# Fantom-foundation/go-txflow

Measured on AMD Instinct MI355X. Metric: verified+tallied TxVotes/sec, higher is better.
Workload: dtype u32

## Files before the change

go-txflow_amd/csrc/kernels_flow.hip:

```cpp
#include <algorithm>

#include "sha2.h"
#include "txv_device.h"
#include "txv_flow.h"
#include "lookback.h"

namespace {

constexpr int64_t kAminoMinSec = -62135596800LL;
constexpr int64_t kAminoMaxSec = 253402300800LL;
constexpr uint64_t kAddrSeed = 0x61646472ULL;
constexpr uint32_t kScanItems = 1024;

__device__ __forceinline__ uint64_t ld64u(const uint8_t* p) {
  const uintptr_t a = (uintptr_t)p;
  const uint32_t* q = reinterpret_cast<const uint32_t*>(a & ~(uintptr_t)3);
  const uint32_t s = (uint32_t)(a & 3u);
  const uint32_t w0 = q[0], w1 = q[1], w2 = q[2];
  return ((uint64_t)__builtin_amdgcn_alignbyte(w2, w1, s) << 32) | __builtin_amdgcn_alignbyte(w1, w0, s);
}

__device__ __forceinline__ bool key_eq(const uint8_t* a, const uint8_t* b, uint32_t n) {
  uint32_t i = 0;
  for (; i + 8 <= n; i += 8)
    if (ld64u(a + i) != ld64u(b + i)) return false;
  if (i < n) {
    const uint64_t m = (1ull << (8 * (n - i))) - 1ull;
    if ((ld64u(a + i) ^ ld64u(b + i)) & m) return false;
  }
  return true;
}

constexpr uint32_t kKeyRegBytes = 64;
struct KeyRegs {
  uint32_t w[16];
};
__device__ __forceinline__ void load_key(const uint8_t* p, uint32_t n, KeyRegs& k) {
  const uintptr_t a = (uintptr_t)p;
  const uint4* q = reinterpret_cast<const uint4*>(a & ~(uintptr_t)15);
  const uint32_t s = (uint32_t)(a & 15u);
  uint32_t raw[20];
#pragma unroll
  for (int c = 0; c < 5; ++c) {
    const uint4 v = (16u * c < s + n) ? q[c] : make_uint4(0, 0, 0, 0);
    raw[4 * c] = v.x; raw[4 * c + 1] = v.y; raw[4 * c + 2] = v.z; raw[4 * c + 3] = v.w;
// ... 271 lines not shown
  }
  if (t == 0) blk[nb] = total;
}

template <class Pred, class Act>
__global__ void __launch_bounds__(256) txv_k_scan_apply(Pred p, Act act, uint32_t n, const uint32_t* blk) {
  __shared__ uint32_t cnt[4][4];
  const uint32_t base = blockIdx.x * kScanItems + threadIdx.x;
  const int lane = threadIdx.x & 63, w = threadIdx.x >> 6;
  bool f[4];
  uint64_t m[4];
#pragma unroll
  for (int k = 0; k < 4; ++k) {
    f[k] = base + 256u * k < n && p(base + 256u * k);
    m[k] = __ballot(f[k]);
    if (lane == 0) cnt[k][w] = (uint32_t)__popcll(m[k]);
  }
  __syncthreads();
  uint32_t rank = blk[blockIdx.x];
  const uint64_t below = (1ull << lane) - 1ull;
#pragma unroll
  for (int k = 0; k < 4; ++k) {
    uint32_t before = 0, round = 0;
#pragma unroll
    for (int q = 0; q < 4; ++q) {
      before += q < w ? cnt[k][q] : 0u;
      round += cnt[k][q];
    }
    if (f[k]) act(base + 256u * k, rank + before + (uint32_t)__popcll(m[k] & below));
    rank += round;
  }
}

struct NewSetPred {
  FlowState fs;
  FlowBatch b;
  __device__ bool operator()(uint32_t i) const {
    const uint32_t e = b.entry[i];
    if (e == TXV_NONE) return false;
    const SetEntry& s = fs.tab[e];
    return s.state == TXV_SE_BATCH && s.first == i;
  }
};

struct NewSetAct {
  FlowState fs;
  FlowBatch b;
  __device__ void operator()(uint32_t i, uint32_t rank) const {
    const uint32_t slot = b.entry[i];
    SetEntry& e = fs.tab[slot];
    const uint32_t id = fs.ctr->n_sets + rank;
    e.state = TXV_SE_KEPT;
    if (id >= fs.max_txs) {
      atomicOr(&fs.ctr->err, TXV_FERR_SETS);
      e.id = TXV_NONE;
      return;
    }
    const uint32_t len = e.len, span = (len + 7u) & ~7u;
    uint64_t ko = (uint64_t)id * TXV_KEY_SLOT;
    if (len > TXV_KEY_SLOT) {
      const unsigned long long o = atomicAdd((unsigned long long*)&fs.ctr->key_used, (unsigned long long)span);
      if (o + span + 16 > fs.keys_cap) {
        atomicOr(&fs.ctr->err, TXV_FERR_KEYS);
        e.id = TXV_NONE;
        return;
      }
      ko = (uint64_t)fs.max_txs * TXV_KEY_SLOT + o;
    }
    const uint8_t* src = b.th + (e.key_off - 1);
    uint64_t* dst = reinterpret_cast<uint64_t*>(fs.keys + ko);
    for (uint32_t k = 0; k < span; k += 8)
      dst[k / 8] = ld64u(src + k) & (k + 8 <= len ? ~0ull : ((1ull << (8 * (len - k))) - 1ull));
    e.key_off = ko + 1;
    e.id = id;
    fs.set_entry[id] = slot;
    uint32_t* tk = fs.set_txkey + (size_t)id * 8;
    if (b.txkey) {
      const uint4* s4 = reinterpret_cast<const uint4*>(b.txkey + (size_t)i * 32);
      const uint4 a = s4[0], c = s4[1];
      tk[0] = a.x; tk[1] = a.y; tk[2] = a.z; tk[3] = a.w; tk[4] = c.x; tk[5] = c.y; tk[6] = c.z; tk[7] = c.w;
    } else {
#pragma unroll
      for (int j = 0; j < 8; ++j) tk[j] = 0;
    }
  }
};

__device__ __forceinline__ uint64_t cand_key(uint32_t stamp, uint32_t i) {
  return ((uint64_t)(0xFFFFFFFFu - stamp) << 32) | i;
}
__device__ __forceinline__ uint32_t cand_of(uint64_t c, uint32_t stamp) {
  return (uint32_t)(c >> 32) == 0xFFFFFFFFu - stamp ? (uint32_t)c : TXV_NONE;
}

constexpr uint8_t kReadCell = 1;
__global__ void __launch_bounds__(256) txv_k_tally_min(FlowState fs, FlowBatch b, uint32_t nb) {
  const uint32_t i = blockIdx.x * 256 + threadIdx.x;
  if (i == 0) {
    const uint32_t created = b.blk[nb];
    const uint32_t ns = fs.ctr->n_sets + created;
    fs.ctr->n_sets = ns > fs.max_txs ? fs.max_txs : ns;
    fs.ctr->n_stamped = 0;
    fs.ctr->ev_ticket = 0;
  }
  if (i >= b.n) return;
  const uint32_t e = b.entry[i];
  const uint32_t s = e == TXV_NONE ? TXV_NONE : fs.tab[e].id;
  b.set[i] = s;
  if (s == TXV_NONE || b.pre[i] != TXV_S_PENDING) return;
  if (b.ok[i] != 1) { b.status[i] = kReadCell; return; }
  TallyCell& c = fs.cell[(size_t)s * fs.n_vals + b.val[i]];
  if (c.acc != 0) { b.status[i] = kReadCell; return; }
  const uint64_t key = cand_key(b.stamp, i);
  const uint64_t old = atomicMin((unsigned long long*)&c.cand, (unsigned long long)key);
  uint8_t tf = 0;
  if (old < key) tf = kReadCell;
  else if (cand_of(old, b.stamp) != TXV_NONE) b.mark[(uint32_t)old] = 1;
  b.status[i] = tf;
}

__device__ __forceinline__ bool pending_in_set(const FlowBatch& b, uint32_t i) {
  return b.pre[i] == TXV_S_PENDING && b.set[i] != TXV_NONE;
}

__device__ __forceinline__ bool sig_eq_arena(const FlowState& fs, const FlowBatch& b, uint32_t i, uint32_t r) {
  uint32_t d = 0;
#pragma unroll
  for (int j = 0; j < 16; ++j) d |= b.sig[(size_t)j * b.n_pad + i] ^ fs.arena_sig[(size_t)j * fs.max_accepted + r];
  return d == 0;
}
__device__ __forceinline__ bool sig_eq_votes(const FlowBatch& b, uint32_t i, uint32_t f) {
  uint32_t d = 0;
// ... 208 lines not shown
    b.ev_host[rank] = e;
  }
};

__global__ void __launch_bounds__(256) txv_k_status_out(FlowState fs, FlowBatch b) {
  const uint32_t base = blockIdx.x * kScanItems + threadIdx.x;
  uint32_t c = 0;
#pragma unroll
  for (int k = 0; k < 4; ++k) {
    const uint32_t i = base + 256u * k;
    if (i >= b.n) continue;
    const uint8_t p = b.pre[i];
    uint8_t st = p;
    if (p == TXV_S_PENDING) {
      const uint32_t s = b.set[i];
      if (s == TXV_NONE) {
        st = TXV_S_INVALID_SIGNATURE;
      } else {
        st = b.status[i];
        if (st == TXV_S_ADDED) {
          const uint32_t x = fs.set_cross[s];
          if (x != TXV_NO_CROSS && i >= x) st |= TXV_S_FIRED;
        }
      }
    }
    b.status_host[i] = st;
    c += b.ev_flag[i] != 0;
  }
  uint32_t total;
  (void)block_excl_scan(c, &total);
  if (threadIdx.x == 0) b.blk[blockIdx.x] = total;
}

__global__ void __launch_bounds__(256) txv_k_event_top(FlowState fs, FlowBatch b, uint32_t nb) {
  const uint32_t t = threadIdx.x;
  const uint32_t per = (nb + 255) / 256;
  const uint32_t lo = min(t * per, nb), hi = min(lo + per, nb);
  uint32_t s = 0;
  for (uint32_t j = lo; j < hi; ++j) s += b.blk[j];
  uint32_t total;
  uint32_t run = block_excl_scan(s, &total);
  for (uint32_t j = lo; j < hi; ++j) {
    const uint32_t v = b.blk[j];
    b.blk[j] = run;
    run += v;
  }
  if (t == 0) {
    b.blk[nb] = total;
    FlowSummary sm;
    sm.n_sets = fs.ctr->n_sets;
    sm.n_events = total;
    sm.arena_used = min(fs.ctr->arena_used, fs.max_accepted);
    sm.err = fs.ctr->err;
    sm.key_used = fs.ctr->key_used;
    *b.summary_host = sm;
  }
}

constexpr uint32_t kFusedEventTiles = 128;
__global__ void __launch_bounds__(256) txv_k_status_events(FlowState fs, FlowBatch b, uint32_t n_tiles) {
  const uint32_t tile = take_tile(&fs.ctr->ev_ticket);
  const uint32_t base = tile * kScanItems + threadIdx.x;
  bool f[4];
#pragma unroll
  for (int k = 0; k < 4; ++k) {
    const uint32_t i = base + 256u * k;
    f[k] = false;
    if (i >= b.n) continue;
    const uint8_t p = b.pre[i];
    uint8_t st = p;
    if (p == TXV_S_PENDING) {
      const uint32_t s = b.set[i];
      if (s == TXV_NONE) {
        st = TXV_S_INVALID_SIGNATURE;
      } else {
        st = b.status[i];
        if (st == TXV_S_ADDED) {
          const uint32_t x = fs.set_cross[s];
          if (x != TXV_NO_CROSS && i >= x) st |= TXV_S_FIRED;
        }
      }
    }
    b.status_host[i] = st;
    f[k] = b.ev_flag[i] != 0;
  }
  uint32_t rank[4], total;
  tile_scan(f, rank, b.ev_tiles, tile, b.stamp, &fs.ctr->err, TXV_FERR_LOOKBACK, &total);
#pragma unroll
  for (int k = 0; k < 4; ++k) {
    if (!f[k]) continue;
    const uint32_t i = base + 256u * k, s = b.set[i];
    FlowEvent e;
    e.vote_index = i;
    e.tx_index = s;
    e.sum = fs.set_sum[s];
    b.ev_host[rank[k]] = e;
  }
  if (tile + 1 == n_tiles && threadIdx.x == 0) {
    FlowSummary sm;
    sm.n_sets = fs.ctr->n_sets;
    sm.n_events = total;
    sm.arena_used = min(fs.ctr->arena_used, fs.max_accepted);
    sm.err = __hip_atomic_load(&fs.ctr->err, __ATOMIC_RELAXED, __HIP_MEMORY_SCOPE_AGENT);
    sm.key_used = fs.ctr->key_used;
    *b.summary_host = sm;
  }
}

__global__ void __launch_bounds__(256) txv_k_reset_sets(FlowState fs, int keep_ids) {
  const uint32_t ns = fs.ctr->n_sets;
  const uint64_t cells = (uint64_t)ns * fs.n_vals;
  const uint64_t stride = (uint64_t)gridDim.x * 256;
  for (uint64_t c = (uint64_t)blockIdx.x * 256 + threadIdx.x; c < cells; c += stride)
    *reinterpret_cast<uint64_t*>(&fs.cell[c].acc) = 0;
  for (uint64_t s = (uint64_t)blockIdx.x * 256 + threadIdx.x; s < ns; s += stride) {
    fs.set_sum[s] = 0;
    if (!keep_ids) {
      SetEntry& e = fs.tab[fs.set_entry[s]];
      e.h = 0; e.len = 0; e.key_off = 0; e.first = 0; e.id = 0; e.state = TXV_SE_EMPTY;
    }
  }
}

__global__ void __launch_bounds__(256) txv_k_init_cells(FlowState fs, uint64_t cells, int clear_acc) {
  const uint64_t stride = (uint64_t)gridDim.x * 256;
  for (uint64_t c = (uint64_t)blockIdx.x * 256 + threadIdx.x; c < cells; c += stride) {
    fs.cell[c].cand = ~0ull;
    if (clear_acc) *reinterpret_cast<uint64_t*>(&fs.cell[c].acc) = 0;
  }
}

__global__ void txv_k_reset_counters(FlowState fs, int keep_ids) {
  if (!keep_ids) {
    fs.ctr->n_sets = 0;
    fs.ctr->n_digested = 0;
    fs.ctr->key_used = 0;
    fs.ctr->err = 0;
  } else {
    fs.ctr->err &= ~TXV_FERR_ARENA;
  }
  fs.ctr->arena_used = 0;
}

__global__ void __launch_bounds__(256) txv_k_lookup(FlowState fs, const uint8_t* keys, const uint32_t* off,
                                                    const uint32_t* len, uint32_t n, uint32_t* out_id) {
  const uint32_t q = blockIdx.x * 256 + threadIdx.x;
  if (q >= n) return;
  const uint8_t* kp = keys + off[q];
  const uint32_t l = len[q];
  const uint64_t h = txv_hash::hash_chunks(l, fs.hash_seed, [&](uint32_t k) { return ld64u(kp + k); });
  uint32_t id = TXV_NONE;
  for (uint32_t slot = (uint32_t)h & fs.tab_mask, probes = 0; probes <= fs.tab_mask; slot = (slot + 1) & fs.tab_mask, ++probes) {
    const SetEntry& e = fs.tab[slot];
    if (e.state == TXV_SE_EMPTY) break;
    if (e.state == TXV_SE_KEPT && e.h == h && e.len == l && key_eq(fs.keys + (e.key_off - 1), kp, l)) {
      id = e.id;
      break;
    }
  }
  out_id[q] = id;
}

__global__ void __launch_bounds__(256) txv_k_gather(FlowState fs, const uint32_t* ids, uint32_t n, int64_t* out_sum,
                                                    uint32_t* out_txkey, AccRow* out_rows) {
  const uint64_t t = (uint64_t)blockIdx.x * 256 + threadIdx.x;
  const uint32_t q = (uint32_t)(t / fs.n_vals), v = (uint32_t)(t % fs.n_vals);
  if (q >= n) return;
  const uint32_t id = ids[q];
  const bool ok = id != TXV_NONE && id < fs.max_txs;
  if (v == 0) {
    if (out_sum) out_sum[q] = ok ? fs.set_sum[id] : 0;
    if (out_txkey)
      for (int j = 0; j < 8; ++j) out_txkey[(size_t)q * 8 + j] = ok ? fs.set_txkey[(size_t)id * 8 + j] : 0u;
  }
// ... 44 lines not shown
  for (int j = 0; j < 4; ++j) fs.set_digest[(size_t)id * 4 + j] = __builtin_bswap32(h[j]);
}

__global__ void __launch_bounds__(256) txv_k_pack(FlowState fs, uint32_t* dst, uint32_t bm_words, uint32_t n_cap) {
  const uint32_t t = blockIdx.x * 256 + threadIdx.x;
  const uint32_t ns = min(fs.ctr->n_sets, n_cap);
  if (t == 0) { dst[0] = ns; dst[1] = 1; fs.ctr->n_digested = ns; }
  if (t < bm_words) dst[2 + t] = commit_word(fs, t, ns);
  if (t < n_cap) {
    const int64_t sm = t < ns ? fs.set_sum[t] : 0;
    dst[2 + bm_words + 2 * t] = (uint32_t)(uint64_t)sm;
    dst[2 + bm_words + 2 * t + 1] = (uint32_t)((uint64_t)sm >> 32);
    uint32_t* dg = dst + 2 + bm_words + 2 * (size_t)n_cap + 4 * (size_t)t;
#pragma unroll
    for (int j = 0; j < 4; ++j) dg[j] = t < ns ? fs.set_digest[(size_t)t * 4 + j] : 0u;
  }
}

__global__ void __launch_bounds__(256) txv_k_bitmap(FlowState fs, uint32_t* dst, uint32_t bm_words) {
  const uint32_t t = blockIdx.x * 256 + threadIdx.x;
  if (t < bm_words) dst[t] = commit_word(fs, t, min(fs.ctr->n_sets, fs.max_txs));
}

constexpr uint32_t kStampCompactMin = 1u << 18;
struct StampPred {
  FlowState fs;
  FlowBatch b;
  __device__ bool operator()(uint32_t s) const { return fs.set_stamp[s] == b.stamp; }
};
struct StampAct {
  FlowBatch b;
  __device__ void operator()(uint32_t s, uint32_t rank) const { b.stamped[rank] = s; }
};

template <class Pred, class Act>
hipError_t compact(Pred p, Act act, uint32_t n, uint32_t* blk, hipStream_t st) {
  const uint32_t nb = (n + kScanItems - 1) / kScanItems;
  if (nb) hipLaunchKernelGGL((txv_k_scan_count<Pred>), dim3(nb), dim3(256), 0, st, p, n, blk);
  hipLaunchKernelGGL(txv_k_scan_top, dim3(1), dim3(256), 0, st, blk, nb);
  if (nb) hipLaunchKernelGGL((txv_k_scan_apply<Pred, Act>), dim3(nb), dim3(256), 0, st, p, act, n, blk);
  return hipGetLastError();
}

#ifdef TXV_EXP_SKIP
uint32_t exp_skip() {
  static const uint32_t m = getenv("TXV_EXP_SKIP") ? (uint32_t)strtoul(getenv("TXV_EXP_SKIP"), nullptr, 0) : 0u;
  return m;
}
#define TXV_SKIP(bit) (exp_skip() & (bit))
#else
#define TXV_SKIP(bit) false
#endif

}

extern "C" {

hipError_t txv_flow_prep(const FlowState* fs, const FlowBatch* b, hipStream_t st) {
  if (((uint64_t)b->n + kScanItems - 1) / kScanItems > 8192) return hipErrorInvalidValue;
  const uint32_t g = (b->n + 255) / 256;
  if (g) hipLaunchKernelGGL(txv_k_route_prep, dim3(g), dim3(256), 0, st, *fs, *b);
  return hipGetLastError();
}

hipError_t txv_flow_route(const FlowState* fs, const FlowBatch* b, hipStream_t st) {
  if (((uint64_t)b->n + kScanItems - 1) / kScanItems > 8192) return hipErrorInvalidValue;
  const uint32_t g = (b->n + 255) / 256;
  if (g && !TXV_SKIP(64)) hipLaunchKernelGGL(txv_k_route_key, dim3(g), dim3(256), 0, st, *fs, *b);
  return hipGetLastError();
}

hipError_t txv_flow_new_ids(const FlowState* fs, const FlowBatch* b, hipStream_t st) {
  if (TXV_SKIP(128)) return hipSuccess;
  return compact(NewSetPred{*fs, *b}, NewSetAct{*fs, *b}, b->n, b->blk, st);
}

hipError_t txv_flow_tally(const FlowState* fs, const FlowBatch* b, uint32_t sets_bound, hipStream_t st) {
  const uint32_t nb = (b->n + kScanItems - 1) / kScanItems;
  const uint32_t g = (b->n + 255) / 256;
  if (!TXV_SKIP(1)) hipLaunchKernelGGL(txv_k_tally_min, dim3(g ? g : 1), dim3(256), 0, st, *fs, *b, nb);
  sets_bound = std::min(sets_bound, fs->max_txs);
  const bool stamp_only = b->n >= kStampCompactMin;
  if (b->n && !TXV_SKIP(2))
    hipLaunchKernelGGL(txv_k_tally_resolve, dim3((b->n + 1023) / 1024), dim3(1024), 0, st, *fs, *b, stamp_only ? 1 : 0);
  const uint32_t* n_stamped = &fs->ctr->n_stamped;
  if (stamp_only) {
    hipError_t e;
    if ((e = compact(StampPred{*fs, *b}, StampAct{*b}, sets_bound, fs->set_blk, st))) return e;
    n_stamped = fs->set_blk + (sets_bound + kScanItems - 1) / kScanItems;
  }
  static const uint32_t cross_cap = getenv("TXV_CROSS_BLOCKS") ? (uint32_t)atoi(getenv("TXV_CROSS_BLOCKS")) : 4096u;
  const uint32_t cross_blocks = std::max<uint32_t>(1, std::min<uint32_t>(std::min(sets_bound, b->n), cross_cap));
  if (!TXV_SKIP(16)) {
    if (fs->n_vals <= 128) hipLaunchKernelGGL(txv_k_tally_cross<128>, dim3(cross_blocks), dim3(64), 0, st, *fs, *b, n_stamped);
    else hipLaunchKernelGGL(txv_k_tally_cross<kListCap>, dim3(cross_blocks), dim3(64), 0, st, *fs, *b, n_stamped);
  }
  if (TXV_SKIP(32)) return hipGetLastError();
  if (nb <= kFusedEventTiles) {
    const uint32_t n_tiles = nb ? nb : 1u;
    hipLaunchKernelGGL(txv_k_status_events, dim3(n_tiles), dim3(256), 0, st, *fs, *b, n_tiles);
    return hipGetLastError();
  }
  hipLaunchKernelGGL(txv_k_status_out, dim3(nb), dim3(256), 0, st, *fs, *b);
  hipLaunchKernelGGL(txv_k_event_top, dim3(1), dim3(256), 0, st, *fs, *b, nb);
  hipLaunchKernelGGL((txv_k_scan_apply<EventPred, EventAct>), dim3(nb), dim3(256), 0, st, EventPred{*b},
                     EventAct{*fs, *b}, b->n, b->blk);
  return hipGetLastError();
}

__global__ void __launch_bounds__(256) txv_k_fill64(uint64_t* dst, uint64_t v, uint32_t n) {
  const uint32_t i = blockIdx.x * 256 + threadIdx.x;
  if (i < n) dst[i] = v;
}

__device__ __forceinline__ uint32_t hex_nibbles8(uint64_t c) {
  uint32_t out = 0;
#pragma unroll
  for (int k = 0; k < 8; ++k) {
    const uint32_t ch = (uint32_t)(c >> (8 * k)) & 0xFFu;
    const uint32_t nib = ch <= '9' ? ch - '0' : ch - 'A' + 10u;
    out |= nib << ((k & 1) ? 8 * (k >> 1) : 8 * (k >> 1) + 4);
  }
  return out;
}

__global__ void __launch_bounds__(256) txv_k_txkey_from_hash(const uint8_t* th, const uint32_t* off, const uint8_t* nil,
                                                             uint32_t n, uint8_t* txkey) {
  const uint32_t i = blockIdx.x * 256 + threadIdx.x;
  if (i >= n) return;
  uint32_t w[8] = {0, 0, 0, 0, 0, 0, 0, 0};
  if (!(nil && nil[i])) {
    const uint8_t* p = th + off[i];
#pragma unroll
    for (int k = 0; k < 8; ++k) w[k] = hex_nibbles8(ld64u(p + 8 * k));
  }
  uint4* d = reinterpret_cast<uint4*>(txkey + (size_t)i * 32);
  d[0] = make_uint4(w[0], w[1], w[2], w[3]);
  d[1] = make_uint4(w[4], w[5], w[6], w[7]);
}

hipError_t txv_txkey_from_hash(const uint8_t* th, const uint32_t* off, const uint8_t* nil, uint32_t n, uint8_t* txkey,
                               hipStream_t st) {
  if (!n) return hipSuccess;
  hipLaunchKernelGGL(txv_k_txkey_from_hash, dim3((n + 255) / 256), dim3(256), 0, st, th, off, nil, n, txkey);
  return hipGetLastError();
}

hipError_t txv_fill64(uint64_t* dst, uint64_t v, uint32_t n, hipStream_t st) {
  if (!n) return hipSuccess;
  hipLaunchKernelGGL(txv_k_fill64, dim3((n + 255) / 256), dim3(256), 0, st, dst, v, n);
  return hipGetLastError();
}

hipError_t txv_flow_reset(const FlowState* fs, int keep_ids, hipStream_t st) {
  hipLaunchKernelGGL(txv_k_reset_sets, dim3(1024), dim3(256), 0, st, *fs, keep_ids);
  hipLaunchKernelGGL(txv_k_reset_counters, dim3(1), dim3(1), 0, st, *fs, keep_ids);
  return hipGetLastError();
}

hipError_t txv_flow_init_cells(const FlowState* fs, uint64_t cells, int clear_acc, hipStream_t st) {
  if (!cells) return hipSuccess;
  hipLaunchKernelGGL(txv_k_init_cells, dim3((uint32_t)std::min<uint64_t>((cells + 255) / 256, 8192)), dim3(256), 0, st,
                     *fs, cells, clear_acc);
  return hipGetLastError();
}

hipError_t txv_flow_lookup(const FlowState* fs, const uint8_t* keys, const uint32_t* off, const uint32_t* len,
                           uint32_t n, uint32_t* out_id, hipStream_t st) {
  if (!n) return hipSuccess;
  hipLaunchKernelGGL(txv_k_lookup, dim3((n + 255) / 256), dim3(256), 0, st, *fs, keys, off, len, n, out_id);
  return hipGetLastError();
}

hipError_t txv_flow_gather(const FlowState* fs, const uint32_t* ids, uint32_t n, int64_t* out_sum, uint32_t* out_txkey,
                           AccRow* out_rows, hipStream_t st) {
  const uint64_t t = (uint64_t)n * std::max<uint32_t>(fs->n_vals, 1);
  if (!t || !fs->n_vals) return hipSuccess;
  hipLaunchKernelGGL(txv_k_gather, dim3((uint32_t)((t + 255) / 256)), dim3(256), 0, st, *fs, ids, n, out_sum, out_txkey,
                     out_rows);
  return hipGetLastError();
}

hipError_t txv_flow_keys(const FlowState* fs, const uint32_t* ids, uint32_t n, uint64_t* out_off, uint32_t* out_len,
                         hipStream_t st) {
  if (!n) return hipSuccess;
  hipLaunchKernelGGL(txv_k_keys, dim3((n + 255) / 256), dim3(256), 0, st, *fs, ids, n, out_off, out_len);
  return hipGetLastError();
}

// ... 15 lines not shown
```

go-txflow_amd/csrc/runtime.cpp:

```cpp
#include "../../include/txvote.h"
#include "txv_device.h"
#include "txv_flow.h"
#include "amino.hpp"
#include "host_pack.hpp"
#include "sha2.h"
#include "route.h"

#include <hip/hip_runtime.h>
#include <emmintrin.h>
#include <algorithm>
#include <chrono>
#include <cstdio>
#include <cctype>
#include <cstdlib>
#include <sched.h>
#include <cstring>
#include <memory>
#include <mutex>
#include <random>
#include <system_error>
#include <thread>
#include <string>
#include <unordered_map>
#include <vector>
// ... 39 lines not shown
  uint32_t *h_fo = nullptr, *h_fl = nullptr, *d_fo = nullptr, *d_fl = nullptr;
  uint8_t *h_arena = nullptr, *d_arena_th = nullptr;
  size_t arena_cap = 0;
  uint64_t arena_end = 0;
  uint32_t flow_cap = 0;
  uint8_t *h_addr = nullptr, *d_addr = nullptr;
  uint32_t *h_addr_len = nullptr, *d_addr_len = nullptr;
  uint8_t *h_sigraw = nullptr, *d_sigraw = nullptr;
  uint32_t *h_sig_len = nullptr, *d_sig_len = nullptr;
  uint8_t *h_nil = nullptr, *d_nil = nullptr;
  uint8_t *h_txkey = nullptr, *d_txkey = nullptr;
  uint16_t *h_vcode = nullptr, *d_vcode = nullptr;
  bool has_nil = false, has_txkey = false, host_val = false;
  uint32_t fill_mask = 0;
  int64_t fill_h = 0, fill_s = 0;
  uint32_t fill_hl = 0, fill_al = 0, fill_sl = 0;
  bool fill_key = false;
  bool msg_on_device = false;
  uint64_t seq_base = 0;
  uint32_t stamp = 0;
  uint64_t run_seq = 0;
  uint64_t counted = 0;
  uint32_t *d_entry = nullptr, *d_blk = nullptr;
  uint8_t* d_ev_flag = nullptr;
  uint8_t* d_mark = nullptr;
  uint32_t* d_stamped = nullptr;
  uint64_t* d_ev_tiles = nullptr;
  uint32_t ev_tiles_n = 0;
  uint8_t* h_out = nullptr; uint8_t* m_out = nullptr;
  FlowEvent* h_ev = nullptr; FlowEvent* m_ev = nullptr;
  FlowSummary* h_sum = nullptr; FlowSummary* m_sum = nullptr;
  hipEvent_t ev[9] = {nullptr, nullptr, nullptr, nullptr, nullptr, nullptr, nullptr, nullptr, nullptr};
  bool launched = false;
  uint32_t* sink = nullptr;
  uint32_t sink_cap = 0;
  uint64_t ticket = 0;
};

}

struct ErrMsg {
  std::mutex m;
  std::string s;
  ErrMsg& operator=(std::string v) {
    std::lock_guard<std::mutex> g(m);
    s = std::move(v);
    return *this;
  }
  const char* copy() {
    thread_local std::string t;
    std::lock_guard<std::mutex> g(m);
    t = s;
    return t.c_str();
  }
};

struct txv_ctx {
  txv_config cfg{};
  int device = 0;
  int n_cus = 256;
  hipStream_t stream = nullptr;
  hipStream_t vstream = nullptr;
  hipStream_t copy_stream = nullptr;
  hipStream_t key_stream = nullptr;
  hipEvent_t tally_ev = nullptr;
  bool tally_ev_set = false;
// ... 692 lines not shown
    HIP_TRY(c, hipMemcpyAsync(s.d_arena_th + ae, s.h_arena + ae, 16, hipMemcpyHostToDevice, c->copy_stream));
  }
  s.fill_key = derive_key;
  if (route && (r = slot_fills(c, s, c->copy_stream))) return r;
  {
    uint64_t up = ae + 16 + (host_val ? (uint64_t)n * 2 : 0);
    for (int k = 0; k < nc; ++k) up += (uint64_t)n * cols[k].elem;
    c->staged_bytes = up;
  }
  HIP_TRY(c, hipEventRecord(s.ev[3], c->copy_stream));
  ht.mark("upload");
  s.staged = true; s.ran = false;
  return TXV_OK;
}

FlowBatch flow_batch(const txv_ctx* c, const Slot& s) {
  FlowBatch b{};
  b.n = s.n; b.n_pad = s.n_pad; b.msg_words = s.msg_words; b.chain_len = (uint32_t)c->chain.size();
  b.seq_base = s.seq_base;
  b.stamp = s.stamp;
  b.height = s.d_fh; b.ts_sec = s.d_fs; b.ts_nanos = s.d_fn; b.th_off = s.d_fo; b.th_len = s.d_fl; b.th = s.d_arena_th;
  b.addr = s.d_addr; b.addr_len = s.d_addr_len; b.sig_raw = s.d_sigraw; b.sig_len = s.d_sig_len;
  b.nil = s.has_nil ? s.d_nil : nullptr; b.txkey = s.has_txkey ? s.d_txkey : nullptr;
  b.vcode = s.host_val ? s.d_vcode : nullptr;
  b.sig = s.d_sig; b.msg_len = s.d_msg_len; b.val = s.d_val; b.flags = s.d_flags; b.pre = s.d_pre;
  b.entry = s.d_entry; b.set = s.d_set; b.ok = s.d_ok; b.status = s.d_status;
  b.ev_flag = s.d_ev_flag; b.mark = s.d_mark; b.blk = s.d_blk; b.stamped = s.d_stamped; b.ev_tiles = s.d_ev_tiles;
  b.status_host = s.m_out; b.ev_host = s.m_ev; b.summary_host = s.m_sum;
  return b;
}

int slot_kernel_ms(txv_ctx* c, Slot& s, float* ms) {
  float k1a = 0.f, k1b = 0.f;
  if (TXV_K1A_ON_KEY_STREAM) {
    HIP_TRY(c, hipEventElapsedTime(&ms[0], s.ev[0], s.ev[8]));
    HIP_TRY(c, hipEventElapsedTime(&k1a, s.ev[8], s.ev[1]));
  } else {
    HIP_TRY(c, hipEventElapsedTime(&ms[0], s.ev[0], s.ev[1]));
  }
  HIP_TRY(c, hipEventElapsedTime(&k1b, s.ev[7], s.ev[2]));
  ms[1] = k1a + k1b;
  HIP_TRY(c, hipEventElapsedTime(&ms[2], s.ev[2], s.ev[5]));
  HIP_TRY(c, hipEventElapsedTime(&ms[3], s.ev[0], s.ev[5]));
  return TXV_OK;
}

int run_slot(txv_ctx* c, uint32_t slot, float* ms) {
  Slot& s = c->slots[slot];
  if (!s.staged) { c->err = "slot not staged"; return TXV_ESTATE; }
  if (c->poisoned) { c->err = "a TxFlow capacity was exceeded: txv_reset_flow first"; return TXV_ECAPACITY; }
  int r;
  if ((r = ensure_park(c))) return r;
  if (c->stamp == 0xFFFFFFFEu) {
    const FlowState fs0 = flow_state(c);
    HIP_TRY(c, txv_flow_init_cells(&fs0, (uint64_t)c->cfg.max_txs * std::max<uint32_t>(c->n_vals, 1), 0, c->stream));
    HIP_TRY(c, hipMemsetAsync(c->d_set_stamp, 0, (size_t)c->cfg.max_txs * 4, c->stream));
    c->stamp = 0;
  }
  s.stamp = ++c->stamp;
  if ((s.stamp & 0x3FFFFFFFu) == 1u)
    for (Slot& o : c->slots)
      if (o.d_ev_tiles) HIP_TRY(c, hipMemsetAsync(o.d_ev_tiles, 0, (size_t)o.ev_tiles_n * sizeof(uint64_t), c->stream));
  s.run_seq = ++c->run_seq;
  const FlowState fs = flow_state(c);
  const FlowBatch fb = flow_batch(c, s);
  hipStream_t ps = c->key_stream;
  HIP_TRY(c, hipStreamWaitEvent(ps, s.ev[3], 0));
  if (s.launched) HIP_TRY(c, hipStreamWaitEvent(ps, s.ev[4], 0));
  if (s.fill_mask || s.fill_key) {
    if ((r = slot_fills(c, s, ps))) return r;
    HIP_TRY(c, hipEventRecord(s.ev[3], ps));
  }
  HIP_TRY(c, hipStreamWaitEvent(c->stream, s.ev[3], 0));
  static const bool prep_after = getenv("TXV_PREP_AFTER_K1B") && atoi(getenv("TXV_PREP_AFTER_K1B")) == 1;
  if (prep_after && c->vend_n >= 2) HIP_TRY(c, hipStreamWaitEvent(ps, c->vend_ev[(c->vend_n - 2) % 4], 0));
  HIP_TRY(c, hipEventRecord(s.ev[0], ps));
  SignBytesArgs sa{};
  sa.n = s.n; sa.n_pad = s.n_pad; sa.msg_words = s.msg_words; sa.chain_len = fb.chain_len;
  sa.height = s.d_fh; sa.ts_sec = s.d_fs; sa.ts_nanos = s.d_fn; sa.txhash_off = s.d_fo; sa.txhash_len = s.d_fl;
  sa.txhash = s.d_arena_th; sa.chain = c->d_chain; sa.msg_len = nullptr; sa.nil = s.has_nil ? s.d_nil : nullptr;
  sa.msg = s.d_msg;
  VerifyArgs va = verify_args(c, s, c->d_pubs, c->d_decode_ok, c->d_atables, c->tab_w, c->d_vslot);
  va.order = nullptr;
  va.n_work = s.n;
  va.lane_votes = launch_lane_votes(c, c->b_w, va.n_work);
  if (!txv_verify_windows_supported(c->b_w, c->tab_w)) { c->err = "verify windows"; return TXV_EDEVICE; }
  static const bool fuse = getenv("TXV_K1B_FUSED") && atoi(getenv("TXV_K1B_FUSED")) == 1;
  va.fused_k1a = fuse && txv_k1b_fusable(c->b_w, &va) ? 1u : 0u;
  HIP_TRY(c, txv_flow_prep(&fs, &fb, ps));
  HIP_TRY(c, txv_launch_signbytes(&sa, ps));
  if (TXV_K1A_ON_KEY_STREAM && !va.fused_k1a) {
    HIP_TRY(c, hipEventRecord(s.ev[8], ps));
    HIP_TRY(c, txv_launch_challenge(&va, ps));
  }
  HIP_TRY(c, hipEventRecord(s.ev[1], ps));
  HIP_TRY(c, hipStreamWaitEvent(c->vstream, s.ev[1], 0));
  HIP_TRY(c, hipEventRecord(s.ev[7], c->vstream));
  static const bool after_tally = getenv("TXV_K1B_AFTER_TALLY") && atoi(getenv("TXV_K1B_AFTER_TALLY")) == 1;
  if (!TXV_K1A_ON_KEY_STREAM || va.fused_k1a) {
    if (!va.fused_k1a) HIP_TRY(c, txv_launch_challenge(&va, c->vstream));
    if (after_tally && c->tally_ev_set) HIP_TRY(c, hipStreamWaitEvent(c->vstream, c->tally_ev, 0));
    HIP_TRY(c, hipEventRecord(s.ev[8], c->vstream));
  }
  HIP_TRY(c, txv_launch_scalarmult(c->b_w, c->tab_w, &va, verify_grid(c, s.n), c->vstream));
  HIP_TRY(c, hipEventRecord(s.ev[2], c->vstream));
  if (prep_after) {
    hipEvent_t& ve = c->vend_ev[c->vend_n % 4];
    if (!ve) HIP_TRY(c, hipEventCreateWithFlags(&ve, hipEventDisableTiming));
    HIP_TRY(c, hipEventRecord(ve, c->vstream));
    ++c->vend_n;
  }
  HIP_TRY(c, txv_flow_route(&fs, &fb, c->stream));
  HIP_TRY(c, txv_flow_new_ids(&fs, &fb, c->stream));
  HIP_TRY(c, hipEventRecord(s.ev[6], c->stream));
  c->unfetched += s.n;
  s.counted += s.n;
  const uint32_t sets_bound = (uint32_t)std::min<uint64_t>((uint64_t)c->n_sets_host + c->unfetched, c->cfg.max_txs);
  HIP_TRY(c, hipStreamWaitEvent(c->stream, s.ev[2], 0));
  HIP_TRY(c, txv_flow_tally(&fs, &fb, sets_bound, c->stream));
  HIP_TRY(c, hipEventRecord(s.ev[5], c->stream));
  if (after_tally) {
    if (!c->tally_ev) HIP_TRY(c, hipEventCreateWithFlags(&c->tally_ev, hipEventDisableTiming));
    HIP_TRY(c, hipEventRecord(c->tally_ev, c->stream));
    c->tally_ev_set = true;
  }
  if (s.sink) HIP_TRY(c, txv_flow_pack(&fs, s.sink, (s.sink_cap + 31) / 32, s.sink_cap, c->stream));
  HIP_TRY(c, hipEventRecord(s.ev[4], c->stream));
  s.ran = true;
  s.launched = true;
  if (ms) {
    HIP_TRY(c, hipEventSynchronize(s.ev[4]));
    if ((r = slot_kernel_ms(c, s, ms))) return r;
// ... 1033 lines not shown
  HIP_TRY(c, hipSetDevice(c->device));
  return fetch_slot(c, slot, status_out, ev, ev_cap, n_ev);
}

int txv_set_commit_sink(txv_ctx* c, uint32_t slot, void* dst_dev, uint32_t n_sets_cap) {
  if (!c || slot >= kStagedSlots || (dst_dev && !n_sets_cap)) return TXV_EINVAL;
  std::lock_guard<std::mutex> g(c->mu);
  HIP_TRY(c, hipSetDevice(c->device));
  Slot& s = c->slots[slot];
  if (s.ticket) { c->err = "slot holds a txv_submit_votes batch in flight"; return TXV_ESTATE; }
  if (s.launched) HIP_TRY(c, hipEventSynchronize(s.ev[4]));
  s.sink = static_cast<uint32_t*>(dst_dev);
  s.sink_cap = dst_dev ? n_sets_cap : 0;
  return TXV_OK;
}

int txv_slot_kernel_ms(txv_ctx* c, uint32_t slot, float* ms4) {
  if (!c || !ms4 || slot >= kStagedSlots) return TXV_EINVAL;
  std::lock_guard<std::mutex> g(c->mu);
  HIP_TRY(c, hipSetDevice(c->device));
  Slot& s = c->slots[slot];
  if (!s.launched) { c->err = "slot never ran"; return TXV_ESTATE; }
  HIP_TRY(c, hipEventSynchronize(s.ev[4]));
  return slot_kernel_ms(c, s, ms4);
}

int txv_slot_verify_ms(txv_ctx* c, uint32_t slot, float* ms2) {
  if (!c || !ms2 || slot >= kStagedSlots) return TXV_EINVAL;
  std::lock_guard<std::mutex> g(c->mu);
  HIP_TRY(c, hipSetDevice(c->device));
  Slot& s = c->slots[slot];
  if (!s.launched) { c->err = "slot never ran"; return TXV_ESTATE; }
  HIP_TRY(c, hipEventSynchronize(s.ev[4]));
  if (TXV_K1A_ON_KEY_STREAM) {
    HIP_TRY(c, hipEventElapsedTime(&ms2[0], s.ev[8], s.ev[1]));
    HIP_TRY(c, hipEventElapsedTime(&ms2[1], s.ev[7], s.ev[2]));
  } else {
    HIP_TRY(c, hipEventElapsedTime(&ms2[0], s.ev[7], s.ev[8]));
    HIP_TRY(c, hipEventElapsedTime(&ms2[1], s.ev[8], s.ev[2]));
  }
  return TXV_OK;
}

int txv_commit_bitmap(txv_ctx* c, void** dev_ptr, uint64_t* bytes) {
  if (!c || !dev_ptr || !bytes) return TXV_EINVAL;
  std::lock_guard<std::mutex> g(c->mu);
  HIP_TRY(c, hipSetDevice(c->device));
  if (!c->d_ctr) { c->err = "no validator set"; return TXV_ESTATE; }
  const FlowState fs = flow_state(c);
  HIP_TRY(c, txv_flow_bitmap(&fs, c->d_bitmap, (c->cfg.max_txs + 31) / 32, c->stream));
  HIP_TRY(c, hipStreamSynchronize(c->stream));
  *dev_ptr = c->d_bitmap;
  *bytes = (uint64_t)(c->cfg.max_txs + 31) / 32 * 4;
  return TXV_OK;
}

int txv_host_register(txv_ctx* c, void* ptr, uint64_t bytes) {
  if (!c || !ptr || !bytes) return TXV_EINVAL;
  std::lock_guard<std::mutex> g(c->mu);
  HIP_TRY(c, hipSetDevice(c->device));
  HIP_TRY(c, hipHostRegister(ptr, bytes, hipHostRegisterDefault));
  std::lock_guard<std::mutex> rg(c->reg_mu);
  c->registered.emplace_back((uintptr_t)ptr, bytes);
  return TXV_OK;
}

int txv_host_unregister(txv_ctx* c, void* ptr) {
// ... 1970 lines not shown
```

go-txflow_amd/csrc/txv_flow.h:

```cpp
#pragma once
#include <stdint.h>
#include <hip/hip_runtime.h>

#include "txv_hash.h"

#define TXV_NO_CROSS 0xFFFFFFFFu
#define TXV_NONE 0xFFFFFFFFu

#define TXV_S_ADDED 0u
#define TXV_S_DUPLICATE 1u
#define TXV_S_NIL 2u
#define TXV_S_EMPTY_ADDR 3u
#define TXV_S_UNKNOWN_VALIDATOR 4u
#define TXV_S_NONDETERMINISTIC 5u
#define TXV_S_INVALID_SIGNATURE 6u
#define TXV_S_SIGNBYTES 8u
#define TXV_S_PENDING 0xFFu
#define TXV_S_FIRED 0x80u

#define TXV_FERR_SETS 0x1u
#define TXV_FERR_TABLE 0x2u
#define TXV_FERR_KEYS 0x4u
#define TXV_FERR_ARENA 0x8u
#define TXV_FERR_LOOKBACK 0x10u
// ... 7 lines not shown
#define TXV_SE_EMPTY 0u
#define TXV_SE_BUSY 1u
#define TXV_SE_BATCH 2u
#define TXV_SE_KEPT 3u

struct SetEntry {
  uint64_t h;
  uint32_t state;
  uint32_t len;
  uint64_t key_off;
  uint32_t first;
  uint32_t id;
};
#define TXV_KEY_SLOT 64u

struct AccRow {
  uint32_t sig[16];
  int64_t height;
  int64_t ts_sec;
  int32_t ts_nanos;
  uint32_t val;
  uint64_t seq;
  uint32_t txkey[8];
};

struct FlowCounters {
  uint32_t n_sets;
  uint32_t arena_used;
  uint32_t err;
  uint32_t n_stamped;
  uint32_t n_digested;
  uint32_t ev_ticket;
  uint64_t key_used;
};

struct FlowSummary {
  uint32_t n_sets, n_events, arena_used, err;
  uint64_t key_used;
};

struct FlowEvent {
  uint32_t vote_index, tx_index;
  int64_t sum;
};

struct FlowState {
  SetEntry* tab;
  uint32_t tab_mask;
  uint32_t max_txs;
  uint8_t* keys;
  uint64_t keys_cap;
  uint32_t* set_entry;
  uint32_t* set_txkey;
  int64_t* set_sum;
  uint32_t* set_stamp;
  uint32_t* set_blk;
  uint32_t* set_cross;
  uint32_t* set_digest;
  TallyCell* cell;
  uint32_t* arena_sig;
  int64_t* arena_height;
  int64_t* arena_sec;
  int32_t* arena_nanos;
  uint32_t* arena_val;
  uint64_t* arena_seq;
  uint32_t* arena_txkey;
// ... 70 lines not shown
```

Baseline: 791.3 million.

## Fuse scan top-level passes into compaction kernels and merge reset launches

Adds a templated compaction kernel in which each block computes its own prefix by re-summing earlier tile counts (or recounting predicates), which removes the separate single-block top-scan launch. Event compaction, new-set id assignment and small stamp compactions now use it, and the new-set total is passed through a counter field. Reset of sets and counters is merged into one kernel that uses a last-block ticket. These changes cut kernel launches and serialization at the cost of redundant prefix work that grows quadratically with the tile count. A runtime env switch for the k1a stream choice is also added.

Result: no change. 793.2 million, median of 2 (+0.2%).

```diff
diff --git a/go-txflow_amd/csrc/kernels_flow.hip b/go-txflow_amd/csrc/kernels_flow.hip
--- a/go-txflow_amd/csrc/kernels_flow.hip
+++ b/go-txflow_amd/csrc/kernels_flow.hip
@@ -11,6 +11,7 @@
 constexpr int64_t kAminoMaxSec = 253402300800LL;
 constexpr uint64_t kAddrSeed = 0x61646472ULL;
 constexpr uint32_t kScanItems = 1024;
+constexpr uint32_t kMaxScanTiles = 8192;
 
 __device__ __forceinline__ uint64_t ld64u(const uint8_t* p) {
   const uintptr_t a = (uintptr_t)p;
@@ -348,6 +349,43 @@
   }
 }
 
+template <bool kCounted, class Pred, class Act, class Fin>
+__global__ void __launch_bounds__(256) txv_k_compact(Pred p, Act act, Fin fin, uint32_t n, const uint32_t* cnt) {
+  __shared__ uint32_t cnt_s[4][4];
+  const uint32_t base = blockIdx.x * kScanItems + threadIdx.x;
+  const int lane = threadIdx.x & 63, w = threadIdx.x >> 6;
+  uint32_t c = 0;
+  if constexpr (kCounted) {
+    for (uint32_t j = threadIdx.x; j < blockIdx.x; j += 256) c += cnt[j];
+  } else {
+    for (uint32_t j = threadIdx.x; j < blockIdx.x * kScanItems; j += 256) c += p(j) ? 1u : 0u;
+  }
+  uint32_t rank;
+  (void)block_excl_scan(c, &rank);
+  bool f[4];
+  uint64_t m[4];
+#pragma unroll
+  for (int k = 0; k < 4; ++k) {
+    f[k] = base + 256u * k < n && p(base + 256u * k);
+    m[k] = __ballot(f[k]);
+    if (lane == 0) cnt_s[k][w] = (uint32_t)__popcll(m[k]);
+  }
+  __syncthreads();
+  const uint64_t below = (1ull << lane) - 1ull;
+#pragma unroll
+  for (int k = 0; k < 4; ++k) {
+    uint32_t before = 0, round = 0;
+#pragma unroll
+    for (int q = 0; q < 4; ++q) {
+      before += q < w ? cnt_s[k][q] : 0u;
+      round += cnt_s[k][q];
+    }
+    if (f[k]) act(base + 256u * k, rank + before + (uint32_t)__popcll(m[k] & below));
+    rank += round;
+  }
+  if (blockIdx.x + 1 == gridDim.x && threadIdx.x == 0) fin(rank);
+}
+
 struct NewSetPred {
   FlowState fs;
   FlowBatch b;
@@ -402,6 +440,11 @@
   }
 };
 
+struct NewSetFin {
+  FlowState fs;
+  __device__ void operator()(uint32_t total) const { fs.ctr->n_new = total; }
+};
+
 __device__ __forceinline__ uint64_t cand_key(uint32_t stamp, uint32_t i) {
   return ((uint64_t)(0xFFFFFFFFu - stamp) << 32) | i;
 }
@@ -413,7 +456,7 @@
 __global__ void __launch_bounds__(256) txv_k_tally_min(FlowState fs, FlowBatch b, uint32_t nb) {
   const uint32_t i = blockIdx.x * 256 + threadIdx.x;
   if (i == 0) {
-    const uint32_t created = b.blk[nb];
+    const uint32_t created = nb ? fs.ctr->n_new : 0u;
     const uint32_t ns = fs.ctr->n_sets + created;
     fs.ctr->n_sets = ns > fs.max_txs ? fs.max_txs : ns;
     fs.ctr->n_stamped = 0;
@@ -688,21 +731,10 @@
   if (threadIdx.x == 0) b.blk[blockIdx.x] = total;
 }
 
-__global__ void __launch_bounds__(256) txv_k_event_top(FlowState fs, FlowBatch b, uint32_t nb) {
-  const uint32_t t = threadIdx.x;
-  const uint32_t per = (nb + 255) / 256;
-  const uint32_t lo = min(t * per, nb), hi = min(lo + per, nb);
-  uint32_t s = 0;
-  for (uint32_t j = lo; j < hi; ++j) s += b.blk[j];
-  uint32_t total;
-  uint32_t run = block_excl_scan(s, &total);
-  for (uint32_t j = lo; j < hi; ++j) {
-    const uint32_t v = b.blk[j];
-    b.blk[j] = run;
-    run += v;
-  }
-  if (t == 0) {
-    b.blk[nb] = total;
+struct EventFin {
+  FlowState fs;
+  FlowBatch b;
+  __device__ void operator()(uint32_t total) const {
     FlowSummary sm;
     sm.n_sets = fs.ctr->n_sets;
     sm.n_events = total;
@@ -711,7 +743,7 @@
     sm.key_used = fs.ctr->key_used;
     *b.summary_host = sm;
   }
-}
+};
 
 constexpr uint32_t kFusedEventTiles = 128;
 __global__ void __launch_bounds__(256) txv_k_status_events(FlowState fs, FlowBatch b, uint32_t n_tiles) {
@@ -763,7 +795,8 @@
   }
 }
 
-__global__ void __launch_bounds__(256) txv_k_reset_sets(FlowState fs, int keep_ids) {
+__global__ void __launch_bounds__(256) txv_k_reset(FlowState fs, int keep_ids) {
+  __shared__ uint32_t ticket_s;
   const uint32_t ns = fs.ctr->n_sets;
   const uint64_t cells = (uint64_t)ns * fs.n_vals;
   const uint64_t stride = (uint64_t)gridDim.x * 256;
@@ -776,17 +809,11 @@
       e.h = 0; e.len = 0; e.key_off = 0; e.first = 0; e.id = 0; e.state = TXV_SE_EMPTY;
     }
   }
-}
-
-__global__ void __launch_bounds__(256) txv_k_init_cells(FlowState fs, uint64_t cells, int clear_acc) {
-  const uint64_t stride = (uint64_t)gridDim.x * 256;
-  for (uint64_t c = (uint64_t)blockIdx.x * 256 + threadIdx.x; c < cells; c += stride) {
-    fs.cell[c].cand = ~0ull;
-    if (clear_acc) *reinterpret_cast<uint64_t*>(&fs.cell[c].acc) = 0;
-  }
-}
-
-__global__ void txv_k_reset_counters(FlowState fs, int keep_ids) {
+  __syncthreads();
+  if (threadIdx.x == 0) ticket_s = atomicAdd(&fs.ctr->reset_ticket, 1u);
+  __syncthreads();
+  if (ticket_s + 1 != gridDim.x || threadIdx.x != 0) return;
+  fs.ctr->reset_ticket = 0;
   if (!keep_ids) {
     fs.ctr->n_sets = 0;
     fs.ctr->n_digested = 0;
@@ -796,6 +823,14 @@
     fs.ctr->err &= ~TXV_FERR_ARENA;
   }
   fs.ctr->arena_used = 0;
+}
+
+__global__ void __launch_bounds__(256) txv_k_init_cells(FlowState fs, uint64_t cells, int clear_acc) {
+  const uint64_t stride = (uint64_t)gridDim.x * 256;
+  for (uint64_t c = (uint64_t)blockIdx.x * 256 + threadIdx.x; c < cells; c += stride) {
+    fs.cell[c].cand = ~0ull;
+    if (clear_acc) *reinterpret_cast<uint64_t*>(&fs.cell[c].acc) = 0;
+  }
 }
 
 __global__ void __launch_bounds__(256) txv_k_lookup(FlowState fs, const uint8_t* keys, const uint32_t* off,
@@ -906,6 +941,11 @@
   FlowBatch b;
   __device__ void operator()(uint32_t s, uint32_t rank) const { b.stamped[rank] = s; }
 };
+struct StampFin {
+  uint32_t* total;
+  __device__ void operator()(uint32_t t) const { *total = t; }
+};
+constexpr uint32_t kStampRecountTiles = 64;
 
 template <class Pred, class Act>
 hipError_t compact(Pred p, Act act, uint32_t n, uint32_t* blk, hipStream_t st) {
@@ -931,14 +971,14 @@
 extern "C" {
 
 hipError_t txv_flow_prep(const FlowState* fs, const FlowBatch* b, hipStream_t st) {
-  if (((uint64_t)b->n + kScanItems - 1) / kScanItems > 8192) return hipErrorInvalidValue;
+  if (((uint64_t)b->n + kScanItems - 1) / kScanItems > kMaxScanTiles) return hipErrorInvalidValue;
   const uint32_t g = (b->n + 255) / 256;
   if (g) hipLaunchKernelGGL(txv_k_route_prep, dim3(g), dim3(256), 0, st, *fs, *b);
   return hipGetLastError();
 }
 
 hipError_t txv_flow_route(const FlowState* fs, const FlowBatch* b, hipStream_t st) {
-  if (((uint64_t)b->n + kScanItems - 1) / kScanItems > 8192) return hipErrorInvalidValue;
+  if (((uint64_t)b->n + kScanItems - 1) / kScanItems > kMaxScanTiles) return hipErrorInvalidValue;
   const uint32_t g = (b->n + 255) / 256;
   if (g && !TXV_SKIP(64)) hipLaunchKernelGGL(txv_k_route_key, dim3(g), dim3(256), 0, st, *fs, *b);
   return hipGetLastError();
@@ -946,7 +986,12 @@
 
 hipError_t txv_flow_new_ids(const FlowState* fs, const FlowBatch* b, hipStream_t st) {
   if (TXV_SKIP(128)) return hipSuccess;
-  return compact(NewSetPred{*fs, *b}, NewSetAct{*fs, *b}, b->n, b->blk, st);
+  const uint32_t nb = (b->n + kScanItems - 1) / kScanItems;
+  if (!nb) return hipSuccess;
+  hipLaunchKernelGGL((txv_k_scan_count<NewSetPred>), dim3(nb), dim3(256), 0, st, NewSetPred{*fs, *b}, b->n, b->blk);
+  hipLaunchKernelGGL((txv_k_compact<true, NewSetPred, NewSetAct, NewSetFin>), dim3(nb), dim3(256), 0, st,
+                     NewSetPred{*fs, *b}, NewSetAct{*fs, *b}, NewSetFin{*fs}, b->n, b->blk);
+  return hipGetLastError();
 }
 
 hipError_t txv_flow_tally(const FlowState* fs, const FlowBatch* b, uint32_t sets_bound, hipStream_t st) {
@@ -959,9 +1004,15 @@
     hipLaunchKernelGGL(txv_k_tally_resolve, dim3((b->n + 1023) / 1024), dim3(1024), 0, st, *fs, *b, stamp_only ? 1 : 0);
   const uint32_t* n_stamped = &fs->ctr->n_stamped;
   if (stamp_only) {
-    hipError_t e;
-    if ((e = compact(StampPred{*fs, *b}, StampAct{*b}, sets_bound, fs->set_blk, st))) return e;
-    n_stamped = fs->set_blk + (sets_bound + kScanItems - 1) / kScanItems;
+    const uint32_t tiles = (sets_bound + kScanItems - 1) / kScanItems;
+    n_stamped = fs->set_blk + tiles;
+    if (tiles && tiles <= kStampRecountTiles) {
+      hipLaunchKernelGGL((txv_k_compact<false, StampPred, StampAct, StampFin>), dim3(tiles), dim3(256), 0, st,
+                         StampPred{*fs, *b}, StampAct{*b}, StampFin{fs->set_blk + tiles}, sets_bound, nullptr);
+    } else {
+      hipError_t e;
+      if ((e = compact(StampPred{*fs, *b}, StampAct{*b}, sets_bound, fs->set_blk, st))) return e;
+    }
   }
   static const uint32_t cross_cap = getenv("TXV_CROSS_BLOCKS") ? (uint32_t)atoi(getenv("TXV_CROSS_BLOCKS")) : 4096u;
   const uint32_t cross_blocks = std::max<uint32_t>(1, std::min<uint32_t>(std::min(sets_bound, b->n), cross_cap));
@@ -976,9 +1027,8 @@
     return hipGetLastError();
   }
   hipLaunchKernelGGL(txv_k_status_out, dim3(nb), dim3(256), 0, st, *fs, *b);
-  hipLaunchKernelGGL(txv_k_event_top, dim3(1), dim3(256), 0, st, *fs, *b, nb);
-  hipLaunchKernelGGL((txv_k_scan_apply<EventPred, EventAct>), dim3(nb), dim3(256), 0, st, EventPred{*b},
-                     EventAct{*fs, *b}, b->n, b->blk);
+  hipLaunchKernelGGL((txv_k_compact<true, EventPred, EventAct, EventFin>), dim3(nb), dim3(256), 0, st, EventPred{*b},
+                     EventAct{*fs, *b}, EventFin{*fs, *b}, b->n, b->blk);
   return hipGetLastError();
 }
 
@@ -1027,8 +1077,7 @@
 }
 
 hipError_t txv_flow_reset(const FlowState* fs, int keep_ids, hipStream_t st) {
-  hipLaunchKernelGGL(txv_k_reset_sets, dim3(1024), dim3(256), 0, st, *fs, keep_ids);
-  hipLaunchKernelGGL(txv_k_reset_counters, dim3(1), dim3(1), 0, st, *fs, keep_ids);
+  hipLaunchKernelGGL(txv_k_reset, dim3(1024), dim3(256), 0, st, *fs, keep_ids);
   return hipGetLastError();
 }
 
diff --git a/go-txflow_amd/csrc/runtime.cpp b/go-txflow_amd/csrc/runtime.cpp
--- a/go-txflow_amd/csrc/runtime.cpp
+++ b/go-txflow_amd/csrc/runtime.cpp
@@ -95,6 +95,7 @@
   FlowSummary* h_sum = nullptr; FlowSummary* m_sum = nullptr;
   hipEvent_t ev[9] = {nullptr, nullptr, nullptr, nullptr, nullptr, nullptr, nullptr, nullptr, nullptr};
   bool launched = false;
+  bool k1a_key = false;
   uint32_t* sink = nullptr;
   uint32_t sink_cap = 0;
   uint64_t ticket = 0;
@@ -853,7 +854,7 @@
 
 int slot_kernel_ms(txv_ctx* c, Slot& s, float* ms) {
   float k1a = 0.f, k1b = 0.f;
-  if (TXV_K1A_ON_KEY_STREAM) {
+  if (s.k1a_key) {
     HIP_TRY(c, hipEventElapsedTime(&ms[0], s.ev[0], s.ev[8]));
     HIP_TRY(c, hipEventElapsedTime(&k1a, s.ev[8], s.ev[1]));
   } else {
@@ -864,6 +865,11 @@
   HIP_TRY(c, hipEventElapsedTime(&ms[2], s.ev[2], s.ev[5]));
   HIP_TRY(c, hipEventElapsedTime(&ms[3], s.ev[0], s.ev[5]));
   return TXV_OK;
+}
+
+bool k1a_on_key_stream() {
+  static const bool on = getenv("TXV_K1A_KEY_STREAM") ? atoi(getenv("TXV_K1A_KEY_STREAM")) == 1 : TXV_K1A_ON_KEY_STREAM != 0;
+  return on;
 }
 
 int run_slot(txv_ctx* c, uint32_t slot, float* ms) {
@@ -908,9 +914,10 @@
   if (!txv_verify_windows_supported(c->b_w, c->tab_w)) { c->err = "verify windows"; return TXV_EDEVICE; }
   static const bool fuse = getenv("TXV_K1B_FUSED") && atoi(getenv("TXV_K1B_FUSED")) == 1;
   va.fused_k1a = fuse && txv_k1b_fusable(c->b_w, &va) ? 1u : 0u;
+  s.k1a_key = !va.fused_k1a && k1a_on_key_stream();
   HIP_TRY(c, txv_flow_prep(&fs, &fb, ps));
   HIP_TRY(c, txv_launch_signbytes(&sa, ps));
-  if (TXV_K1A_ON_KEY_STREAM && !va.fused_k1a) {
+  if (s.k1a_key) {
     HIP_TRY(c, hipEventRecord(s.ev[8], ps));
     HIP_TRY(c, txv_launch_challenge(&va, ps));
   }
@@ -918,7 +925,7 @@
   HIP_TRY(c, hipStreamWaitEvent(c->vstream, s.ev[1], 0));
   HIP_TRY(c, hipEventRecord(s.ev[7], c->vstream));
   static const bool after_tally = getenv("TXV_K1B_AFTER_TALLY") && atoi(getenv("TXV_K1B_AFTER_TALLY")) == 1;
-  if (!TXV_K1A_ON_KEY_STREAM || va.fused_k1a) {
+  if (!s.k1a_key) {
     if (!va.fused_k1a) HIP_TRY(c, txv_launch_challenge(&va, c->vstream));
     if (after_tally && c->tally_ev_set) HIP_TRY(c, hipStreamWaitEvent(c->vstream, c->tally_ev, 0));
     HIP_TRY(c, hipEventRecord(s.ev[8], c->vstream));
@@ -2018,7 +2025,7 @@
   Slot& s = c->slots[slot];
   if (!s.launched) { c->err = "slot never ran"; return TXV_ESTATE; }
   HIP_TRY(c, hipEventSynchronize(s.ev[4]));
-  if (TXV_K1A_ON_KEY_STREAM) {
+  if (s.k1a_key) {
     HIP_TRY(c, hipEventElapsedTime(&ms2[0], s.ev[8], s.ev[1]));
     HIP_TRY(c, hipEventElapsedTime(&ms2[1], s.ev[7], s.ev[2]));
   } else {
diff --git a/go-txflow_amd/csrc/txv_flow.h b/go-txflow_amd/csrc/txv_flow.h
--- a/go-txflow_amd/csrc/txv_flow.h
+++ b/go-txflow_amd/csrc/txv_flow.h
@@ -63,6 +63,8 @@
   uint32_t n_digested;
   uint32_t ev_ticket;
   uint64_t key_used;
+  uint32_t n_new;
+  uint32_t reset_ticket;
 };
 
 struct FlowSummary {
```
